# qq456cvb/CPPF2

Hardware: AMD Instinct MI355X
Metric: scenes/sec (1/2/4/8 GPU) at 4096 pts x 20k tuples; 5deg5cm match vs ref (higher is better)
Workload: dtype f32

## Files before the change

### cppf2_amd/_lib.py

```python
from __future__ import annotations

import ctypes as C
import os

_PKG = os.path.dirname(os.path.abspath(__file__))
LIB_PATH = os.path.join(_PKG, "libcppf_hip.so")
if os.environ.get("CPPF_LIB"):
    LIB_PATH = os.path.abspath(os.environ["CPPF_LIB"])

ABI_VERSION = 11


class CppfError(RuntimeError):
    pass


class SceneGrid(C.Structure):
    _fields_ = [("c0", C.c_float * 3), ("g", C.c_int32 * 3), ("ncell", C.c_int32), ("flags", C.c_int32)]


class SceneResult(C.Structure):
    _fields_ = [("argmax", C.c_int64), ("t", C.c_double * 3), ("R", C.c_double * 9), ("scale", C.c_float * 3),
                ("peak", C.c_uint32), ("up_idx", C.c_int32), ("right_idx", C.c_int32), ("kept", C.c_int32),
                ("up_count", C.c_float), ("right_count", C.c_float), ("flags", C.c_int32), ("ncell", C.c_int32), ("pad_", C.c_int32 * 3)]


class ReslayerSplit16Args(C.Structure):
    _fields_ = [("x", C.c_void_p), ("ldx", C.c_int64), ("k_in", C.c_int32),
                ("out", C.c_void_p), ("ldo", C.c_int64), ("n_out", C.c_int32), ("rows", C.c_int64),
                ("wq", C.c_void_p), ("wq_bytes", C.c_int64), ("b1", C.c_void_p), ("b0", C.c_void_p), ("chain", C.c_int32),
                ("weight_scale", C.c_float),
                ("first_out", C.c_void_p), ("ld_first", C.c_int64),
                ("gidx", C.c_void_p), ("slots", C.c_int32), ("table", C.c_void_p), ("fdim", C.c_int32),
                ("logit_prior", C.c_void_p), ("uniforms", C.c_void_p), ("bins", C.c_void_p),
                ("stream", C.c_void_p), ("mode", C.c_int32), ("ld_table", C.c_int64), ("sched", C.c_void_p),
                ("prior_pos", C.c_void_p), ("prior_inv_sigma", C.c_float)]


assert C.sizeof(SceneGrid) == 32
assert C.sizeof(SceneResult) == 160

_p = C.c_void_p
_i = C.c_int
_i32 = C.c_int32
_i64 = C.c_int64
_u64 = C.c_uint64
_f = C.c_float
_d = C.c_double

STABLE = {
    "cppf_version": (_i, []),
    "cppf_last_error_string": (C.c_char_p, []),
# ... 49 lines not shown
}

EXPERIMENTAL = {
    "cppf_shot352_from_normals": (_i, [_i, _p, _p, _i64, _p, _f, _p, _p, _p, _i64, _p]),
    "cppf_cast_f16": (_i, [_p, _p, _i64, _p]),
    "cppf_encode_tuples_shot_f16": (_i, [_i, _p, _p, _p, _i, _p, _i, _p, _p, _i64, _p, _p]),
    "cppf_encode_tuples_dino": (_i, [_i, _p, _i, _i, _p, _p, _p, _p, _i64, _p, _i, _i, _p]),
    "cppf_kept_rows": (_i, [_i, _p, _p, _p, _i, _p, _p]),
    "cppf_reslayer128": (_i, [_p, _i64, _p, _p, _p, _p]),
    "cppf_encode_tuples_shot_heads": (_i, [_i, _p, _p, _p, _i, _p, _p, _i64, _p, _i, _p, _p]),
    "cppf_reslayer_split_gather": (_i, [_p, _i64, _i, _p, _i, _p, _i, _p, _i64, _i, _i64, _p, _i64, _p, _p, _i, _p, _p]),
    "cppf_encode_tuples_coord_heads": (_i, [_i, _p, _p, _i, _p, _p, _i64, _p, _i32, _p, _p]),
    "cppf_reslayer_split_sumgather": (_i, [_p, _i64, _i32, _p, _i32, _p, _i64, _p, _i64, _i32, _i64, _p, _i64, _p, _p, _i32, _p, _p]),
    "cppf_reslayer_split16_stream_bytes": (_i64, [_i32, _i32, _i32, _i32]),
    "cppf_reslayer_split16": (_i, [_p]),
    "cppf_reslayer_split_debug_grid": (_i, [_i32]),
    "cppf_decode_bins_prior": (_i, [_i, _p, _p, _i, _p, _p, _p, _i, _p, _p, _i64, _p, _p, _p, _p, _p, _p, _p]),
    "cppf_reslayer_split_decode_prior": (_i, [_p, _i64, _i, _i64, _p, _i64, _p, _p, _p, _p, C.c_float, _p, _p, _p, _p]),
}

SIGNATURES = dict(STABLE, **EXPERIMENTAL)

CALLED = set()


class _Traced:
    def __init__(self, lib):
        self._lib = lib
        for name in SIGNATURES:
            setattr(self, name, self._wrap(name, getattr(lib, name)))
# ... 42 lines not shown
```

### cppf2_amd/csrc/cppf_mlp_split.hip

```cpp
#include "cppf_common.h"
#include <atomic>
#include <mutex>
#include <type_traits>

typedef float f32x16 __attribute__((ext_vector_type(16)));
typedef float f32x4 __attribute__((ext_vector_type(4)));
typedef __bf16 bf16x8 __attribute__((ext_vector_type(8)));

__host__ __device__ constexpr int rs_waves(int nt) { return nt >= 6 ? 4 : 8; }
#define RS_RESLAYER 0
#define RS_LINEAR 1
#define RS_SUMGATHER 2
#define RS_ENCODE 3
#define RS_SUMENCODE 5
__host__ __device__ constexpr int rs_waves_mode(int nt, int mode) { return mode == RS_LINEAR ? 8 : rs_waves(nt); }
__host__ __device__ constexpr int rs_stage_tiles(int mode) { return 16; }
__host__ __device__ constexpr int rs_wgs_per_cu(int mode) { return 1; }
#define RS_FRAG_BYTES 1024
__host__ __device__ constexpr int rs_stage_bytes(int stg) { return stg * 3 * RS_FRAG_BYTES; }
__host__ __device__ constexpr int rs_tile_bytes(int pc) { return pc * RS_FRAG_BYTES; }

#ifndef RS_DEEP_PREFETCH
#define RS_DEEP_PREFETCH 0
#endif
// ... 73 lines not shown
  acc = rs_mfma<PC>(a.l, b.h, acc);
  acc = rs_mfma<PC>(a.h, b.l, acc);
  if (PC == 3) {
    acc = rs_mfma<PC>(a.m, b.m, acc);
    acc = rs_mfma<PC>(a.m, b.h, acc);
    acc = rs_mfma<PC>(a.h, b.m, acc);
  }
  acc = rs_mfma<PC>(a.h, b.h, acc);
}

__host__ __device__ constexpr int rs_waitcnt(int vm, int lgkm) {
  return (vm & 15) | ((vm >> 4) << 14) | (7 << 4) | ((lgkm & 15) << 8);
}
#define RS_WAIT(vm, lgkm) __builtin_amdgcn_s_waitcnt(rs_waitcnt(vm, lgkm))

template <int NT, int T0, int WAVES, int PC, bool LIN = false, int STG = 16>
struct RsStream {
  static constexpr int STG_ = STG, SPC0 = rs_spc(T0, STG), SPC1 = rs_spc(NT, STG), STAGE_BYTES = rs_stage_bytes(STG);
  static constexpr int P0 = (SPC0 * T0 * PC + WAVES - 1) / WAVES, P1 = (SPC1 * NT * PC + WAVES - 1) / WAVES;
  static constexpr int PMAX = RS_EXACT_PMAX ? (P0 > P1 ? P0 : P1) : 48 / WAVES;
  int nseg;
  int chunks;
  const char* base;
  char* ring;
  int ks1;
  int seg, pos;
  int64_t off;
  int64_t left;
  int stage;
  int wave, lane;
  const char* p_src;
  char* p_dst;
  int p_last;

  __device__ __forceinline__ void shape(int chain) {
    if (LIN) {
      nseg = chain;
      chunks = chain * ((ks1 + SPC0 - 1) / SPC0);
      return;
    }
    nseg = 2 + 2 * chain;
    chunks = (ks1 + SPC0 - 1) / SPC0 + (1 + 2 * chain) * (2 * NT / SPC1);
  }
  __device__ __forceinline__ void plan(int st) {
    p_dst = ring + st * STAGE_BYTES;
    if (left <= 0) {
      p_src = base + lane * 16;
      p_last = 0;
      return;
    }
    const bool first = LIN || seg == 0;
    const int tiles = first ? T0 : NT;
    const int spc = first ? SPC0 : SPC1;
    const int steps = first ? ks1 : 2 * NT;
    const int ns = steps - pos < spc ? steps - pos : spc;
    const int pieces = ns * tiles * PC;
    p_src = base + off + lane * 16;
    p_last = pieces - 1;
    off += (int64_t)pieces * RS_FRAG_BYTES;
    pos += ns;
    if (pos == steps) {
      pos = 0;
      if (++seg == nseg) {
        seg = 0;
        off = 0;
      }
    }
    --left;
  }
// ... 146 lines not shown
      const int step = c * SPC + i, nx = (step + 1 < 2 * NS) ? step + 1 : step;
      RsFrag bn = b;
      rs_step<NTILES, PREFETCH, Stream::PMAX, PC>(dst, w + i * NTILES * PC * 64, b,
                                [&](int p) {
                                  if (step + 1 < 2 * NS) {
                                    const float s0 = src[nx >> 1][8 * (nx & 1) + 2 * p], s1 = src[nx >> 1][8 * (nx & 1) + 2 * p + 1];
                                    rs_split_pair<PC, true>(PC == 2 ? s0 * bs : s0, PC == 2 ? s1 * bs : s1, bn.h[p], bn.m[p], bn.l[p]);
                                  }
                                },
                                [&](int q) { if (i == 0) ws.piece(q); });
      b = bn;
    }
  }
}

__device__ __forceinline__ void rs_load_tile(f32x16& acc, const float* v, int g) {
#pragma unroll
  for (int q = 0; q < 4; ++q) {
    const f32x4 t = *reinterpret_cast<const f32x4*>(v + 8 * q + 4 * g);
    acc[4 * q + 0] = t.x; acc[4 * q + 1] = t.y; acc[4 * q + 2] = t.z; acc[4 * q + 3] = t.w;
  }
}

__device__ __forceinline__ void rs_load_tile_scaled(f32x16& acc, const float* v, int g, float sc) {
#pragma unroll
  for (int q = 0; q < 4; ++q) {
    const f32x4 t = *reinterpret_cast<const f32x4*>(v + 8 * q + 4 * g);
    acc[4 * q + 0] = t.x * sc; acc[4 * q + 1] = t.y * sc; acc[4 * q + 2] = t.z * sc; acc[4 * q + 3] = t.w * sc;
  }
}
// ... 175 lines not shown
#pragma unroll
    for (int c = 0; c < 3; ++c) v[3 * q + c] = p[PI_[q]][c] - p[PJ_[q]][c];
  v[30] = 0.0f; v[31] = 0.0f;
#pragma unroll
  for (int s = 0; s < 2; ++s) {
    f32x4 lo, hi;
    lo.x = g ? v[16 * s + 8] : v[16 * s + 0]; lo.y = g ? v[16 * s + 9] : v[16 * s + 1];
    lo.z = g ? v[16 * s + 10] : v[16 * s + 2]; lo.w = g ? v[16 * s + 11] : v[16 * s + 3];
    hi.x = g ? v[16 * s + 12] : v[16 * s + 4]; hi.y = g ? v[16 * s + 13] : v[16 * s + 5];
    hi.z = g ? v[16 * s + 14] : v[16 * s + 6]; hi.w = g ? v[16 * s + 15] : v[16 * s + 7];
    *reinterpret_cast<f32x4*>(slots + s * 2048 + lane * 16) = lo;
    *reinterpret_cast<f32x4*>(slots + s * 2048 + 1024 + lane * 16) = hi;
  }
}

template <int NT, bool PROJ, bool GATHER, bool DECODE = false, int PC = 3, int MODE = RS_RESLAYER>
__global__ __launch_bounds__(64 * rs_waves_mode(NT, MODE), rs_wgs_per_cu(MODE)) void reslayer_split_kernel(const float* x, int64_t ldx, int k_in, float* out,
                                                                              int64_t ldo, int64_t rows,
                                                                              const char* __restrict__ wq,
                                                                              const float* __restrict__ b1,
                                                                              const float* __restrict__ b0, int chain,
                                                                              RsGather ga, RsDecode dc, RsTap tap, float wscale) {
  const float bs = (PC == 2) ? 1.0f / wscale : 1.0f;
  constexpr int WAVES = rs_waves_mode(NT, MODE), THREADS = 64 * WAVES, BLOCK_ROWS = 32 * WAVES;
  constexpr int T0 = PROJ ? 2 * NT : NT;
  constexpr bool LIN = MODE == RS_LINEAR;
  static_assert(!LIN || (!PROJ && !GATHER && !DECODE), "a plain Linear has one product");
  constexpr bool SUMG = MODE == RS_SUMGATHER || MODE == RS_SUMENCODE;
  constexpr bool LOCAL_IDX = MODE == RS_ENCODE || MODE == RS_SUMENCODE;
  static_assert(!SUMG || (PROJ && !GATHER), "the table sums stand for columns of a projection layer's input");
  static_assert(MODE != RS_ENCODE || (GATHER && !DECODE), "RS_ENCODE is a form of the gathering launch");
  constexpr bool PF = RS_DEEP_PREFETCH && WAVES == 4;
  extern __shared__ __attribute__((aligned(16))) char s_ring[];
  const int lane = threadIdx.x & 63;
  const int wave = __builtin_amdgcn_readfirstlane(threadIdx.x >> 6);
  const int r = lane & 31, g = lane >> 5;
  const int ks1 = (k_in + 15) >> 4;
  const int64_t nblocks = (rows + BLOCK_ROWS - 1) / BLOCK_ROWS;
  int64_t bfirst = blockIdx.x, bstride = gridDim.x, bend = nblocks;
  if (RS_XCD_BLOCKS && (gridDim.x & 7) == 0 && nblocks >= 64) {
    const int64_t xcd = blockIdx.x & 7;
    bfirst = nblocks * xcd / 8 + (blockIdx.x >> 3);
    bend = nblocks * (xcd + 1) / 8;
    bstride = gridDim.x >> 3;
  }
  int* const sched = ga.sched;
  const bool dyn = sched != nullptr && !LIN;
  int* const s_claim = reinterpret_cast<int*>(s_ring + 2 * rs_stage_bytes(rs_stage_tiles(MODE)) + WAVES * 3 * 2048 + (2 + chain) * 32 * NT * 4);
  if (dyn) { bfirst = blockIdx.x; bstride = 0; bend = nblocks; }
  const int64_t mine = dyn ? (bfirst < bend ? 1 : 0) : (bend > bfirst ? (bend - bfirst + bstride - 1) / bstride : 0);
  if (dyn && threadIdx.x == 0) rs_claim_store(&s_claim[0], (int)gridDim.x + atomicAdd(&sched[0], 1));

  constexpr int STG = rs_stage_tiles(MODE), RING_BYTES = 2 * rs_stage_bytes(STG);
  RsStream<NT, T0, WAVES, PC, LIN, STG> ws;
  const int64_t seg_bytes = (int64_t)ks1 * T0 * rs_tile_bytes(PC);
  if (LIN) {
    wq += (int64_t)blockIdx.y * chain * seg_bytes;
    b1 = b1 ? b1 + (int64_t)blockIdx.y * chain * 32 * NT : b1;
    out += (int64_t)blockIdx.y * chain * 32 * NT;
  }
  ws.base = wq;
  ws.ring = s_ring;
  ws.ks1 = ks1;
  ws.seg = 0;
  ws.pos = 0;
  ws.off = 0;
  ws.shape(chain);
  ws.left = mine * ws.chunks;
  ws.stage = 0;
  ws.wave = wave;
  ws.lane = lane;
  ws.prime();
  float* s_b1 = reinterpret_cast<float*>(s_ring + RING_BYTES + WAVES * 3 * 2048);
  float* s_b0 = s_b1 + 32 * NT;
  if (LIN) {
    for (int i = threadIdx.x; i < 32 * NT * chain; i += THREADS) s_b1[i] = b1 ? b1[i] : 0.0f;
  } else {
    for (int i = threadIdx.x; i < 32 * NT; i += THREADS) {
      s_b1[i] = b1[i];
      if (PROJ) s_b0[i] = b0[i];
    }
    for (int i = threadIdx.x; i < 32 * NT * chain; i += THREADS) s_b1[2 * 32 * NT + i] = b1[32 * NT + i];
  }
  __syncthreads();

  RsX<GATHER> xs;
  xs.slots = s_ring + RING_BYTES + wave * (3 * 2048);
  xs.k_in = k_in;
  xs.g = g;
  xs.lane = lane;
  xs.table = ga.table;
  xs.head = ga.head;
  xs.fshift = ga.fshift;
  auto row_of = [&](int64_t blk) {
    const int64_t row = blk * BLOCK_ROWS + wave * 32 + r;
    const int64_t rc = row < rows ? row : rows - 1;
    RsRow rw;
// ... 167 lines not shown
      }
    }
#pragma unroll 1
    for (int l = 0; l < chain; ++l) {
      const float* bl = s_b1 + 32 * NT * (2 + l);
#pragma unroll
      for (int u = 0; u < NT; ++u) rs_load_tile(h[u], bl + 32 * u, g);
      rs_product_h<NT, NT, PF, PC>(h, o, ws, bs);
#pragma unroll
      for (int u = 0; u < NT; ++u) {
#pragma unroll
        for (int e = 0; e < 16; ++e) h[u][e] = (h[u][e] < 0.0f) ? 0.0f : h[u][e];
      }
      rs_product_h<NT, NT, PF, PC>(o, h, ws, bs);
    }
    if (DECODE) {
      if constexpr (NT == 6) rs_decode_epilogue<NT, PC>(o, dc, in ? row : rows - 1, in, g, bs);
    } else if (in && (!(RS_DBG & 32) || o[0][0] == 1.2345e30f)) {
      float* orow = out + row * ldo + 4 * g;
#pragma unroll
      for (int u = 0; u < NT; ++u) {
#pragma unroll
        for (int q = 0; q < 4; ++q) {
          f32x4 v;
          v.x = o[u][4 * q + 0]; v.y = o[u][4 * q + 1]; v.z = o[u][4 * q + 2]; v.w = o[u][4 * q + 3];
          if (PC == 2) v *= bs;
          *reinterpret_cast<f32x4*>(orow + 32 * u + 8 * q) = v;
        }
      }
    }
    blk = nb;
    if (dyn) {
      next_blk = rs_claim_load(&s_claim[par]);
      par ^= 1;
    }
  }
  RS_WAIT(0, 15);
  if (dyn && threadIdx.x == 0) {
    if (atomicAdd(&sched[1], 1) == (int)gridDim.x - 1) {
      __hip_atomic_store(&sched[0], 0, __ATOMIC_RELAXED, __HIP_MEMORY_SCOPE_AGENT);
      __hip_atomic_store(&sched[1], 0, __ATOMIC_RELAXED, __HIP_MEMORY_SCOPE_AGENT);
    }
  }
}

static int64_t rs_stream_bytes(int32_t k_in, int32_t n_out, int32_t proj, int32_t chain, int pc) {
  if (k_in <= 0 || !(n_out == 64 || n_out == 128 || n_out == 192 || n_out == 256) || chain < 0 || chain > 15) return -1;
  const int64_t nt = n_out / 32, ks1 = (k_in + 15) / 16;
  return (ks1 * (proj ? 2 : 1) + (1 + 2 * (int64_t)chain) * 2 * nt) * nt * rs_tile_bytes(pc);
}

extern "C" int64_t cppf_reslayer_split_stream_bytes(int32_t k_in, int32_t n_out, int32_t proj, int32_t chain) {
  return rs_stream_bytes(k_in, n_out, proj, chain, 3);
}

static std::atomic<int> g_rs_debug_cus{0};
extern "C" int cppf_reslayer_split_debug_grid(int32_t workgroups) {
  g_rs_debug_cus.store(workgroups > 0 ? workgroups : 0);
  return CPPF_OK;
}

static std::atomic<int> g_rs_reserved_cus{0};
extern "C" int cppf_mlp_reserve_cus(int32_t cus) {
  CPPF_CHECK_ARG(cus <= 1024);
  return cus < 0 ? g_rs_reserved_cus.load() : g_rs_reserved_cus.exchange(cus);
}

template <int NT, bool PROJ, bool GATHER = false, bool DECODE = false, int PC = 3, int MODE = RS_RESLAYER>
static int rs_launch(const float* x, int64_t ldx, int k_in, float* out, int64_t ldo, int64_t rows, const char* wq,
                     const float* b1, const float* b0, int chain, int cus, hipStream_t stream, RsGather ga = RsGather(),
                     RsDecode dc = RsDecode(), RsTap tap = RsTap(), float wscale = 1.0f) {
  constexpr int WAVES = rs_waves_mode(NT, MODE), THREADS = 64 * WAVES, BLOCK_ROWS = 32 * WAVES;
  const int64_t nblocks = (rows + BLOCK_ROWS - 1) / BLOCK_ROWS;
  const int forced = g_rs_debug_cus.load();
  if (forced > 0) cus = forced;
  else cus = cus - g_rs_reserved_cus.load() > cus / 2 ? cus - g_rs_reserved_cus.load() : (cus + 1) / 2;
  cus *= rs_wgs_per_cu(MODE);
  const unsigned grid = (unsigned)(nblocks < cus ? nblocks : cus);
  unsigned gy = 1;
  if (MODE == RS_LINEAR && (int64_t)grid * 2 <= cus) {
    for (int d = chain; d >= 1; --d)
      if (chain % d == 0 && (int64_t)grid * d <= cus) { gy = (unsigned)d; break; }
    chain /= (int)gy;
  }
  const int lds_bytes = 2 * rs_stage_bytes(rs_stage_tiles(MODE)) + WAVES * 3 * 2048 + (MODE == RS_LINEAR ? chain : 2 + chain) * 32 * NT * 4 + 16;
  if (lds_bytes > 160 * 1024 / rs_wgs_per_cu(MODE)) {
    snprintf(g_cppf_err, sizeof(g_cppf_err), "reslayer_split: %d bytes of LDS for the biases of this launch (too many column groups)", lds_bytes);
    return CPPF_EINVAL;
  }
  {
    static std::mutex mu;
    static bool done[64] = {false};
    int dev = 0;
    CPPF_HIP(hipGetDevice(&dev));
    std::lock_guard<std::mutex> lock(mu);
    if (!done[dev & 63]) {
      CPPF_HIP(hipFuncSetAttribute((const void*)reslayer_split_kernel<NT, PROJ, GATHER, DECODE, PC, MODE>,
                                   hipFuncAttributeMaxDynamicSharedMemorySize, 160 * 1024));
      done[dev & 63] = true;
    }
  }
  hipLaunchKernelGGL((reslayer_split_kernel<NT, PROJ, GATHER, DECODE, PC, MODE>), dim3(grid, gy), dim3(THREADS), lds_bytes, stream, x,
                     ldx, k_in, out, ldo, rows, wq, b1, b0, chain, ga, dc, tap, wscale);
  CPPF_LAUNCH_CHECK();
  return CPPF_OK;
}

static int rs_cus() {
  int dev = 0, n_cu = 0;
  if (hipGetDevice(&dev) != hipSuccess || hipDeviceGetAttribute(&n_cu, hipDeviceAttributeMultiprocessorCount, dev) != hipSuccess) return 256;
  return n_cu > 0 ? n_cu : 256;
}

static int rs_dispatch(const float* x, int64_t ldx, int32_t k_in, float* out, int64_t ldo, int32_t n_out, int64_t rows,
                       const void* wq, int64_t wq_bytes, const float* b1, const float* b0, int32_t chain, RsTap tap,
                       int32_t* sched, void* stream, const char* fn) {
  if (!(x && out && wq && b1 && rows >= 0) || !(k_in > 0 && (k_in & 7) == 0 && ldx >= k_in && (ldx & 3) == 0 && (ldo & 3) == 0 && ldo >= n_out) ||
      !(n_out == 64 || n_out == 128 || n_out == 192 || n_out == 256) || !(b0 != nullptr || k_in == n_out) ||
// ... 209 lines not shown
  if (rows == 0) return CPPF_OK;
  RsGather ga;
  ga.gidx = idx;
  ga.table = tables;
  ga.slots = k;
  ga.tld = ld_tables;
  ga.pts = pts;
  ga.pt_off = pt_off;
  ga.tup_off = tup_off;
  ga.B = B;
  ga.sched = sched;
  return rs_launch<4, true, false, false, 3, RS_SUMENCODE>(nullptr, 0, 32, out, ldo, rows, static_cast<const char*>(wq), b1, b0, chain,
                                                           rs_cus(), (hipStream_t)stream, ga);
}

extern "C" int64_t cppf_reslayer_split16_stream_bytes(int32_t k_in, int32_t n_out, int32_t proj, int32_t chain) {
  return rs_stream_bytes(k_in, n_out, proj, chain, 2);
}

static RsGather rs16_gather(const CppfReslayerSplit16Args& a) {
  RsGather ga;
  ga.sched = a.sched;
  return ga;
}

template <int NT, bool PROJ>
static int rs16_plain(const CppfReslayerSplit16Args& a, int n_cu, RsTap tap) {
  return rs_launch<NT, PROJ, false, false, 2>(a.x, a.ldx, a.k_in, a.out, a.ldo, a.rows, static_cast<const char*>(a.wq), a.b1, a.b0,
                                              a.chain, n_cu, (hipStream_t)a.stream, rs16_gather(a), RsDecode(), tap, a.weight_scale);
}
// ... 88 lines not shown
```

### cppf2_amd/models.py

```python
from __future__ import annotations

import os
from itertools import combinations

import torch
import torch.nn as nn
import torch.nn.functional as F

from . import ops


class ResLayer(nn.Module):

    def __init__(self, dim_in, dim_out):
        super().__init__()
        self.fc1 = nn.Linear(dim_in, dim_out)
        self.fc2 = nn.Linear(dim_out, dim_out)
        self.fc0 = nn.Linear(dim_in, dim_out) if dim_in != dim_out else None

    def forward(self, x):
        skip = x if self.fc0 is None else self.fc0(x)
        return self.fc2(F.relu(self.fc1(x))) + skip


# ... 136 lines not shown
        if MLP_ARITH == "split16":
            sc = f16_scale(w1t, w0t, w2t, *[w for pair in chain for w in pair])
            wq = pack_split(w1t.t(), None if w0t is None else w0t.t(), w2t.t(), k_in, chain=chain, arith="f16x2", scale=sc)
            hit = (stamp, (wq, (biases * sc).contiguous(), None if b0 is None else (b0 * sc).contiguous(), sc))
        else:
            wq = pack_split(w1t.t(), None if w0t is None else w0t.t(), w2t.t(), k_in, chain=chain)
            hit = (stamp, (wq, biases.contiguous(), b0, 1.0))
        cache[key] = hit
    return hit[1]


def _chain_len(cache, key, stamp, compute):
    hit = cache.get(key)
    if hit is None or hit[0] != stamp:
        hit = (stamp, compute())
        cache[key] = hit
    return hit[1]


def fused_stack(seq, x, keep_input=False, gather=None, decode=None, tail=None):
    tap_at, cross = None, None
    if isinstance(seq, (tuple, list)):
        seq_a, seq_b = seq
        plan_a, c_a = _fused_plan(seq_a)
        assert c_a is None, "the first stack must end in a projection layer"
        plan_b, c = _fused_plan(seq_b)
        plan = plan_a + plan_b
        tap_at = len(plan_a) - 1
        cross = seq_b._fused_plan_cache[0]
        seq = seq_b
# ... 23 lines not shown
            assert _kernel_arith() and w0t is not None and w1t.shape[1] == 128 and k_in % 8 == 0, "table-fed first layer: see sum_supported"
            w1t, w0t = fold.w1_heads.t(), fold.w0_heads.t()
        else:
            k_in = heads.shape[1] + (source.k if source is not None else gidx.shape[1]) * table.shape[1]
            assert _kernel_arith() and w0t is not None and w1t.shape == (k_in, 128), "gathered first layer: see gather_supported"
        cache = _entry_cache(entry)

        def gather_chain():
            n = 0
            while (1 + n < len(plan) and plan[1 + n][2] is None and n < 15 and plan[1 + n][0].shape == (128, 128)):
                n += 1
            n = cut(0, n)
            return 0 if tap_at == 0 else n
        chain = _chain_len(cache, ("gather-chain", k_in, tap_at), cross, gather_chain)
        crossing = tap_at is not None and chain > tap_at
        stamp = (cross if crossing else None, None if fold is None else fold.stamp)
        wq, bb1, bb0, sc = _packed(cache, (k_in, chain, crossing, fold is not None), w1t, w0t, w2t, k_in, plan[1:1 + chain], b1, b0,
                                   stamp=stamp, add=None if fold is None else (fold.b1_add, fold.b0_add))
        if fold is not None and source is not None:
            x = ops.reslayer_split_sumencode(source, table, wq, bb1, bb0, 128, chain=chain)
        elif fold is not None:
            x = ops.reslayer_split_sumgather(heads, gidx, table, wq, bb1, bb0, 128, chain=chain,
                                             scale=sc if MLP_ARITH == "split16" else None)
        elif MLP_ARITH == "split16":
            x = ops.reslayer_split16(heads, wq, bb1, bb0, 128, sc, chain=chain, gather=(gidx, table))
        elif source is not None:
            x = ops.reslayer_split_encode(source, table, wq, bb1, bb0, 128, chain=chain)
        else:
            x = ops.reslayer_split_gather(heads, gidx, table, wq, bb1, bb0, 128, chain=chain)
        li = 1 + chain
# ... 15 lines not shown
        if (_kernel_arith() and x.dtype == torch.float32 and x.stride(1) == 1 and x.stride(0) % 4 == 0
                and x.data_ptr() % 16 == 0 and x.shape[1] >= w1t.shape[0]
                and ops.reslayer_split_supported(x.shape[1], n_out, w0t is not None)):
            cache = _entry_cache(entry)
            ahead = tap_at is not None and tap_at >= li

            def plain_chain(li=li, n_out=n_out, w0t=w0t):
                n = 0
                while (li + 1 + n < len(plan) and plan[li + 1 + n][2] is None and n < 15
                       and plan[li + 1 + n][0].shape == (n_out, n_out)
                       and ops.reslayer_split_supported(x.shape[1], n_out, w0t is not None, n + 1)):
                    n += 1
                return cut(li, n)
            chain = _chain_len(cache, ("chain", x.shape[1], tap_at if ahead else None), cross if ahead else None, plain_chain)
            crossing = tap_at is not None and li <= tap_at < li + chain
            wq, bb1, bb0, sc = _packed(cache, (x.shape[1], chain, crossing), w1t, w0t, w2t, x.shape[1],
                                       plan[li + 1:li + 1 + chain], b1, b0, stamp=cross if crossing else None)
            out = None
            if w0t is None and li == 0 and keep_input:
                out = torch.empty_like(x)
            if w0t is None and out is None and tapped is not None and x.data_ptr() == tapped.data_ptr():
                out = torch.empty_like(x)
            tap_buf = None
            if tap_at == li and chain > 0:
                tap_buf = torch.empty((x.shape[0], n_out), dtype=torch.float32, device=x.device)
                if w0t is None and out is None:
                    out = torch.empty_like(x)
            if MLP_ARITH == "split16":
                x = ops.reslayer_split16(x, wq, bb1, bb0, n_out, sc, out=out, chain=chain, tap=tap_buf)
            else:
# ... 318 lines not shown
```

### cppf2_amd/ops.py

```python
from __future__ import annotations

import ctypes as C
import math

import numpy as np
import torch

from . import _lib
from ._lib import CppfError, SceneGrid, SceneResult

_L = _lib.load()

BMM_SIZE = 100000


def _dev():
    if not torch.cuda.is_available():
        raise CppfError("cppf2_amd needs a HIP device (torch.cuda.is_available() is False); there is no CPU fallback")
    return torch.device("cuda", torch.cuda.current_device())


def _stream():
    return C.c_void_p(torch.cuda.current_stream().cuda_stream)

# ... 391 lines not shown
    assert heads.is_cuda and heads.dtype == torch.float32 and heads.dim() == 2
    assert gidx.dtype == torch.int32 and gidx.is_contiguous() and table.dtype == torch.float32 and table.is_contiguous()
    rows = gidx.shape[0]
    out = torch.empty((rows, n_out), dtype=torch.float32, device=heads.device)
    b1 = b1.contiguous()
    b0 = b0.contiguous()
    assert b1.numel() == (1 + chain) * n_out
    ld_heads = heads.stride(0) if heads.shape[1] else 0
    _lib.check(_L.cppf_reslayer_split_gather(_p(heads if heads.shape[1] else table), ld_heads, heads.shape[1], _p(gidx), gidx.shape[1], _p(table),
                                             table.shape[1], _p(out), out.stride(0), n_out, rows, _p(wq),
                                             wq.numel() * wq.element_size(), _p(b1), _p(b0), int(chain), _sched(), _stream()),
               "cppf_reslayer_split_gather")
    return out


class TupleSource:

    def __init__(self, points, point_idxs_all, normal=None, pt_off=None, tup_off=None):
        dev = _dev()
        self.pts = _t(points, torch.float32, dev)
        self.nrm = None if normal is None else _t(normal, torch.float32, dev)
        self.idx = _t(point_idxs_all, torch.int32, dev)
        T, self.k = self.idx.shape
        if pt_off is None:
            pt_off, tup_off = _offsets([self.pts.shape[0]], dev), _offsets([T], dev)
        self.pt_off, self.tup_off = pt_off, tup_off
        self.B = pt_off.numel() - 1
        npair = self.k * (self.k - 1) // 2
        self.shape = (T, npair * 4 if normal is not None else (npair * 3 + 7) // 8 * 8)

# ... 375 lines not shown
```

### include/cppf_hip_experimental.h

```cpp
#ifndef CPPF_HIP_EXPERIMENTAL_H_
#define CPPF_HIP_EXPERIMENTAL_H_

#include "cppf_hip.h"

#ifdef __cplusplus
extern "C" {
#endif

int cppf_decode_bins_prior(int B, const float* logits, const float* logit_prior, int nb, const float* uniforms,
                           const float* pts, const int32_t* idx, int k, const int32_t* pt_off, const int32_t* tup_off,
                           int64_t total_tuples, const double* h_axes, int32_t* bins, float* scaled, float* scale,
                           float* tr, float* rot, void* stream);
int cppf_reslayer_split_decode_prior(const float* x, int64_t ldx, int32_t k_in, int64_t rows, const void* wq, int64_t wq_bytes,
                                     const float* b1, const float* b0, const float* logit_prior, const float* prior_pos,
                                     float prior_inv_sigma, const float* uniforms, int32_t* bins, int32_t* sched, void* stream);

int cppf_shot352_from_normals(int B, const float* pts, const int32_t* pt_off, int64_t total_points,
                              const float* normals, float shot_r, float* out_shot, float* out_rf,
                              void* workspace, int64_t workspace_bytes, void* stream);

int cppf_cast_f16(const float* x, void* out_half, int64_t n, void* stream);

int cppf_encode_tuples_shot_f16(int B, const float* pts, const float* normals, const void* feat_half, int feat_dim,
                                const int32_t* idx, int k, const int32_t* pt_off, const int32_t* tup_off,
// ... 30 lines not shown
  const void* wq; int64_t wq_bytes; const float* b1; const float* b0; int32_t chain;
  float weight_scale;
  float* first_out; int64_t ld_first;
  const int32_t* gidx; int32_t slots; const float* table; int32_t fdim;
  const float* logit_prior; const float* uniforms; int32_t* bins;
  void* stream;
  int32_t mode;
  int64_t ld_table;
  int32_t* sched;
  const float* prior_pos;
  float prior_inv_sigma;
} CppfReslayerSplit16Args;
int64_t cppf_reslayer_split16_stream_bytes(int32_t k_in, int32_t n_out, int32_t proj, int32_t chain);
int cppf_reslayer_split16(const CppfReslayerSplit16Args* args);

int cppf_reslayer_split_debug_grid(int32_t workgroups);

#ifdef __cplusplus
}
#endif
#endif
```

Baseline: 5279.

## Fuse 128->64 tail residual layer and narrow output head into the reslayer chain kernel

Extends the split-precision residual MLP kernel so that, after its chain of 128-wide residual blocks, it also runs a following 128->64 projection residual layer in the same launch. On gathered rows it can further apply the final 64->3 narrow layer in a scalar FMA epilogue and scatter the results. The goal is to remove separate kernel launches and the global-memory round trips for the intermediate activations. In exchange it adds more weight-stream segments, extra LDS for tail biases, and register pressure from the larger fused body. It is enabled by default through CHAIN_TAILS when the layer shapes match.

```diff
diff --git a/cppf2_amd/_lib.py b/cppf2_amd/_lib.py
--- a/cppf2_amd/_lib.py
+++ b/cppf2_amd/_lib.py
@@ -36,6 +36,17 @@
                 ("stream", C.c_void_p), ("mode", C.c_int32), ("ld_table", C.c_int64), ("sched", C.c_void_p),
                 ("prior_pos", C.c_void_p), ("prior_inv_sigma", C.c_float)]
 
+
+
+class ReslayerSplitChainArgs(C.Structure):
+    _fields_ = [("x", C.c_void_p), ("ldx", C.c_int64), ("k_in", C.c_int32),
+                ("gidx", C.c_void_p), ("slots", C.c_int32), ("table", C.c_void_p), ("fdim", C.c_int32),
+                ("n_out", C.c_int32), ("n_tail", C.c_int32), ("rows", C.c_int64),
+                ("wq", C.c_void_p), ("wq_bytes", C.c_int64), ("b1", C.c_void_p), ("b0", C.c_void_p), ("chain", C.c_int32),
+                ("out", C.c_void_p), ("ldo", C.c_int64),
+                ("n_narrow", C.c_int32), ("narrow_w", C.c_void_p),
+                ("scatter_rows", C.c_void_p), ("valid_count", C.c_void_p), ("per_group", C.c_int32),
+                ("sched", C.c_void_p), ("stream", C.c_void_p)]
 
 assert C.sizeof(SceneGrid) == 32
 assert C.sizeof(SceneResult) == 160
@@ -115,6 +126,7 @@
     "cppf_reslayer_split_sumgather": (_i, [_p, _i64, _i32, _p, _i32, _p, _i64, _p, _i64, _i32, _i64, _p, _i64, _p, _p, _i32, _p, _p]),
     "cppf_reslayer_split16_stream_bytes": (_i64, [_i32, _i32, _i32, _i32]),
     "cppf_reslayer_split16": (_i, [_p]),
+    "cppf_reslayer_split_chain": (_i, [_p]),
     "cppf_reslayer_split_debug_grid": (_i, [_i32]),
     "cppf_decode_bins_prior": (_i, [_i, _p, _p, _i, _p, _p, _p, _i, _p, _p, _i64, _p, _p, _p, _p, _p, _p, _p]),
     "cppf_reslayer_split_decode_prior": (_i, [_p, _i64, _i, _i64, _p, _i64, _p, _p, _p, _p, C.c_float, _p, _p, _p, _p]),
diff --git a/cppf2_amd/csrc/cppf_mlp_split.hip b/cppf2_amd/csrc/cppf_mlp_split.hip
--- a/cppf2_amd/csrc/cppf_mlp_split.hip
+++ b/cppf2_amd/csrc/cppf_mlp_split.hip
@@ -111,11 +111,17 @@
 }
 #define RS_WAIT(vm, lgkm) __builtin_amdgcn_s_waitcnt(rs_waitcnt(vm, lgkm))
 
-template <int NT, int T0, int WAVES, int PC, bool LIN = false, int STG = 16>
+__host__ __device__ constexpr int rs_pieces(int tiles, int waves, int pc, int stg) {
+  return tiles > 0 ? (rs_spc(tiles, stg) * tiles * pc + waves - 1) / waves : 0;
+}
+__host__ __device__ constexpr int rs_max(int a, int b) { return a > b ? a : b; }
+template <int NT, int T0, int WAVES, int PC, bool LIN = false, int STG = 16, int NT2 = 0>
 struct RsStream {
   static constexpr int STG_ = STG, SPC0 = rs_spc(T0, STG), SPC1 = rs_spc(NT, STG), STAGE_BYTES = rs_stage_bytes(STG);
+  static constexpr int SPC2 = rs_spc(NT2 > 0 ? 2 * NT2 : 1, STG), SPC3 = rs_spc(NT2 > 0 ? NT2 : 1, STG);
   static constexpr int P0 = (SPC0 * T0 * PC + WAVES - 1) / WAVES, P1 = (SPC1 * NT * PC + WAVES - 1) / WAVES;
-  static constexpr int PMAX = RS_EXACT_PMAX ? (P0 > P1 ? P0 : P1) : 48 / WAVES;
+  static constexpr int P23 = rs_max(rs_pieces(2 * NT2, WAVES, PC, STG), rs_pieces(NT2, WAVES, PC, STG));
+  static constexpr int PMAX = RS_EXACT_PMAX ? rs_max(P0 > P1 ? P0 : P1, P23) : 48 / WAVES;
   int nseg;
   int chunks;
   const char* base;
@@ -136,8 +142,9 @@
       chunks = chain * ((ks1 + SPC0 - 1) / SPC0);
       return;
     }
-    nseg = 2 + 2 * chain;
+    nseg = 2 + 2 * chain + (NT2 > 0 ? 2 : 0);
     chunks = (ks1 + SPC0 - 1) / SPC0 + (1 + 2 * chain) * (2 * NT / SPC1);
+    if (NT2 > 0) chunks += 2 * NT / SPC2 + 2 * NT2 / SPC3;
   }
   __device__ __forceinline__ void plan(int st) {
     p_dst = ring + st * STAGE_BYTES;
@@ -147,9 +154,15 @@
       return;
     }
     const bool first = LIN || seg == 0;
-    const int tiles = first ? T0 : NT;
-    const int spc = first ? SPC0 : SPC1;
-    const int steps = first ? ks1 : 2 * NT;
+    int tiles = first ? T0 : NT;
+    int spc = first ? SPC0 : SPC1;
+    int steps = first ? ks1 : 2 * NT;
+    if (NT2 > 0 && seg >= nseg - 2) {
+      const bool w2 = seg == nseg - 1;
+      tiles = w2 ? NT2 : 2 * NT2;
+      spc = w2 ? SPC3 : SPC2;
+      steps = w2 ? 2 * NT2 : 2 * NT;
+    }
     const int ns = steps - pos < spc ? steps - pos : spc;
     const int pieces = ns * tiles * PC;
     p_src = base + off + lane * 16;
@@ -326,6 +339,109 @@
   }
 }
 
+__device__ __forceinline__ void rs_x_order(float (&v)[8], const f32x16& t, int q, int g) {
+#pragma unroll
+  for (int c = 0; c < 4; ++c) {
+    const float a = t[4 * q + c], b = t[4 * q + 4 + c];
+    const float pa = __shfl_xor(a, 32), pb = __shfl_xor(b, 32);
+    v[c] = g ? pb : a;
+    v[4 + c] = g ? b : pa;
+  }
+}
+
+template <int NS, int NTILES, bool PREFETCH, int PC, class Stream>
+__device__ __forceinline__ void rs_product_hx(f32x16 (&dst)[NTILES], const f32x16 (&src)[NS], Stream& ws, int g) {
+  static_assert(PC == 3, "bf16 triples only");
+  constexpr int SPC = rs_spc(NTILES, Stream::STG_);
+  static_assert((2 * NS) % SPC == 0, "whole chunks");
+  float xv[8];
+  rs_x_order(xv, src[0], 0, g);
+  RsFrag b = rs_split<PC>(xv);
+#pragma unroll
+  for (int c = 0; c < 2 * NS / SPC; ++c) {
+    const u32x4* w = ws.template acquire<0>();
+#pragma unroll
+    for (int i = 0; i < SPC; ++i) {
+      const int step = c * SPC + i, nx = (step + 1 < 2 * NS) ? step + 1 : step;
+      float nv[8];
+      rs_x_order(nv, src[nx >> 1], 2 * (nx & 1), g);
+      RsFrag bn = b;
+      rs_step<NTILES, PREFETCH, Stream::PMAX, PC>(dst, w + i * NTILES * PC * 64, b,
+                                [&](int p) {
+                                  if (step + 1 < 2 * NS) rs_split_pair<PC, true>(nv[2 * p], nv[2 * p + 1], bn.h[p], bn.m[p], bn.l[p]);
+                                },
+                                [&](int q) { if (i == 0) ws.piece(q); });
+      b = bn;
+    }
+  }
+}
+
+struct RsNarrow {
+  const float* w = nullptr;
+  const int32_t* scatter_rows = nullptr;
+  const int32_t* valid_count = nullptr;
+  int per_group = 0;
+  float* out = nullptr;
+  int64_t ldo = 0;
+};
+
+template <int NS, int N>
+__device__ __forceinline__ void rs_narrow_epilogue(const f32x16 (&y)[NS], const RsNarrow& nw, const float* __restrict__ w, int row, bool in, int g) {
+  constexpr int K = 32 * NS;
+  int opaque = 0;
+  asm volatile("" : "+s"(opaque));
+  const float* w1 = w + opaque;
+  const float* w0 = w1 + N * K;
+  const float* b1 = w0 + N * K;
+  const float* b0 = b1 + N;
+  const float* w2 = b0 + N;
+  float h[N], s[N];
+#pragma unroll
+  for (int n = 0; n < N; ++n) {
+    h[n] = b1[n];
+    s[n] = b0[n];
+  }
+#pragma unroll
+  for (int t = 0; t < NS; ++t) {
+#pragma unroll
+    for (int q = 0; q < 4; ++q) {
+      float x[8];
+#pragma unroll
+      for (int c = 0; c < 4; ++c) {
+        const float v = y[t][4 * q + c], p = __shfl_xor(v, 32);
+        x[c] = g ? p : v;
+        x[4 + c] = g ? v : p;
+      }
+      const int k0 = 32 * t + 8 * q;
+#pragma unroll
+      for (int j = 0; j < 8; ++j) {
+#pragma unroll
+        for (int n = 0; n < N; ++n) {
+          h[n] = fmaf(x[j], w1[n * K + k0 + j], h[n]);
+          s[n] = fmaf(x[j], w0[n * K + k0 + j], s[n]);
+        }
+      }
+      __builtin_amdgcn_sched_barrier(0);
+    }
+  }
+#pragma unroll
+  for (int n = 0; n < N; ++n) h[n] = (h[n] < 0.0f) ? 0.0f : h[n];
+  int64_t dst = row;
+  if (nw.scatter_rows) {
+    if (nw.valid_count && row % nw.per_group >= nw.valid_count[row / nw.per_group]) in = false;
+    dst = in ? (int64_t)nw.scatter_rows[row] : 0;
+  }
+  if (in && g == 0) {
+#pragma unroll
+    for (int n = 0; n < N; ++n) {
+      float o = s[n];
+#pragma unroll
+      for (int m = 0; m < N; ++m) o = fmaf(h[m], w2[n * N + m], o);
+      nw.out[dst * nw.ldo + n] = o;
+    }
+  }
+}
+
 __device__ __forceinline__ void rs_load_tile(f32x16& acc, const float* v, int g) {
 #pragma unroll
   for (int q = 0; q < 4; ++q) {
@@ -531,13 +647,11 @@
   }
 }
 
-template <int NT, bool PROJ, bool GATHER, bool DECODE = false, int PC = 3, int MODE = RS_RESLAYER>
-__global__ __launch_bounds__(64 * rs_waves_mode(NT, MODE), rs_wgs_per_cu(MODE)) void reslayer_split_kernel(const float* x, int64_t ldx, int k_in, float* out,
-                                                                              int64_t ldo, int64_t rows,
-                                                                              const char* __restrict__ wq,
-                                                                              const float* __restrict__ b1,
-                                                                              const float* __restrict__ b0, int chain,
-                                                                              RsGather ga, RsDecode dc, RsTap tap, float wscale) {
+template <int NT, bool PROJ, bool GATHER, bool DECODE, int PC, int MODE, int NT2, int NARROW>
+__device__ __forceinline__ void reslayer_split_body(const float* x, int64_t ldx, int k_in, float* out, int64_t ldo, int64_t rows,
+                                                    const char* __restrict__ wq, const float* __restrict__ b1,
+                                                    const float* __restrict__ b0, int chain, RsGather ga, RsDecode dc, RsTap tap,
+                                                    float wscale, RsNarrow nw, const float* __restrict__ nw_w) {
   const float bs = (PC == 2) ? 1.0f / wscale : 1.0f;
   constexpr int WAVES = rs_waves_mode(NT, MODE), THREADS = 64 * WAVES, BLOCK_ROWS = 32 * WAVES;
   constexpr int T0 = PROJ ? 2 * NT : NT;
@@ -547,6 +661,8 @@
   constexpr bool LOCAL_IDX = MODE == RS_ENCODE || MODE == RS_SUMENCODE;
   static_assert(!SUMG || (PROJ && !GATHER), "the table sums stand for columns of a projection layer's input");
   static_assert(MODE != RS_ENCODE || (GATHER && !DECODE), "RS_ENCODE is a form of the gathering launch");
+  static_assert(NT2 == 0 || (PC == 3 && MODE == RS_RESLAYER && !DECODE && 2 * NT2 <= NT), "a tail layer at most as wide as the launch");
+  static_assert(NARROW == 0 || NT2 > 0, "the narrow epilogue follows a tail layer");
   constexpr bool PF = RS_DEEP_PREFETCH && WAVES == 4;
   extern __shared__ __attribute__((aligned(16))) char s_ring[];
   const int lane = threadIdx.x & 63;
@@ -563,13 +679,14 @@
   }
   int* const sched = ga.sched;
   const bool dyn = sched != nullptr && !LIN;
-  int* const s_claim = reinterpret_cast<int*>(s_ring + 2 * rs_stage_bytes(rs_stage_tiles(MODE)) + WAVES * 3 * 2048 + (2 + chain) * 32 * NT * 4);
+  int* const s_claim = reinterpret_cast<int*>(s_ring + 2 * rs_stage_bytes(rs_stage_tiles(MODE)) + WAVES * 3 * 2048 + (2 + chain) * 32 * NT * 4 +
+                                              2 * 32 * NT2 * 4);
   if (dyn) { bfirst = blockIdx.x; bstride = 0; bend = nblocks; }
   const int64_t mine = dyn ? (bfirst < bend ? 1 : 0) : (bend > bfirst ? (bend - bfirst + bstride - 1) / bstride : 0);
   if (dyn && threadIdx.x == 0) rs_claim_store(&s_claim[0], (int)gridDim.x + atomicAdd(&sched[0], 1));
 
   constexpr int STG = rs_stage_tiles(MODE), RING_BYTES = 2 * rs_stage_bytes(STG);
-  RsStream<NT, T0, WAVES, PC, LIN, STG> ws;
+  RsStream<NT, T0, WAVES, PC, LIN, STG, NT2> ws;
   const int64_t seg_bytes = (int64_t)ks1 * T0 * rs_tile_bytes(PC);
   if (LIN) {
     wq += (int64_t)blockIdx.y * chain * seg_bytes;
@@ -598,6 +715,8 @@
       if (PROJ) s_b0[i] = b0[i];
     }
     for (int i = threadIdx.x; i < 32 * NT * chain; i += THREADS) s_b1[2 * 32 * NT + i] = b1[32 * NT + i];
+    for (int i = threadIdx.x; i < 2 * 32 * NT2; i += THREADS)
+      s_b1[(2 + chain) * 32 * NT + i] = b1[(1 + chain) * 32 * NT + i];
   }
   __syncthreads();
 
@@ -795,7 +914,35 @@
       }
       rs_product_h<NT, NT, PF, PC>(o, h, ws, bs);
     }
-    if (DECODE) {
+    if constexpr (NT2 > 0) {
+      f32x16 (&t1)[2 * NT2] = *reinterpret_cast<f32x16 (*)[2 * NT2]>(&acc[0]);
+      f32x16 (&h2)[NT2] = *reinterpret_cast<f32x16 (*)[NT2]>(&acc[0]);
+      f32x16 (&o2)[NT2] = *reinterpret_cast<f32x16 (*)[NT2]>(&acc[NT2]);
+      const float* bt = s_b1 + 32 * NT * (2 + chain);
+#pragma unroll
+      for (int u = 0; u < 2 * NT2; ++u) rs_load_tile(t1[u], bt + 32 * u, g);
+      rs_product_hx<NT, 2 * NT2, PF, PC>(t1, o, ws, g);
+#pragma unroll
+      for (int u = 0; u < NT2; ++u) {
+#pragma unroll
+        for (int e = 0; e < 16; ++e) h2[u][e] = (h2[u][e] < 0.0f) ? 0.0f : h2[u][e];
+      }
+      rs_product_h<NT2, NT2, PF, PC>(o2, h2, ws, bs);
+      if constexpr (NARROW > 0) {
+        rs_narrow_epilogue<NT2, NARROW>(o2, nw, nw_w, (int)(in ? row : rows - 1), in, g);
+      } else if (in) {
+        float* orow = out + row * ldo + 4 * g;
+#pragma unroll
+        for (int u = 0; u < NT2; ++u) {
+#pragma unroll
+          for (int q = 0; q < 4; ++q) {
+            f32x4 v;
+            v.x = o2[u][4 * q + 0]; v.y = o2[u][4 * q + 1]; v.z = o2[u][4 * q + 2]; v.w = o2[u][4 * q + 3];
+            *reinterpret_cast<f32x4*>(orow + 32 * u + 8 * q) = v;
+          }
+        }
+      }
+    } else if (DECODE) {
       if constexpr (NT == 6) rs_decode_epilogue<NT, PC>(o, dc, in ? row : rows - 1, in, g, bs);
     } else if (in && (!(RS_DBG & 32) || o[0][0] == 1.2345e30f)) {
       float* orow = out + row * ldo + 4 * g;
@@ -825,6 +972,27 @@
   }
 }
 
+template <int NT, bool PROJ, bool GATHER, bool DECODE = false, int PC = 3, int MODE = RS_RESLAYER>
+__global__ __launch_bounds__(64 * rs_waves_mode(NT, MODE), rs_wgs_per_cu(MODE)) void reslayer_split_kernel(const float* x, int64_t ldx, int k_in, float* out,
+                                                                              int64_t ldo, int64_t rows,
+                                                                              const char* __restrict__ wq,
+                                                                              const float* __restrict__ b1,
+                                                                              const float* __restrict__ b0, int chain,
+                                                                              RsGather ga, RsDecode dc, RsTap tap, float wscale) {
+  reslayer_split_body<NT, PROJ, GATHER, DECODE, PC, MODE, 0, 0>(x, ldx, k_in, out, ldo, rows, wq, b1, b0, chain, ga, dc, tap, wscale,
+                                                               RsNarrow(), nullptr);
+}
+
+template <int NT, bool PROJ, bool GATHER, int NT2, int NARROW>
+__global__ __launch_bounds__(64 * rs_waves(NT), 1) void reslayer_split_chain_kernel(const float* x, int64_t ldx, int k_in, float* out, int64_t ldo,
+                                                                                 int64_t rows, const char* __restrict__ wq,
+                                                                                 const float* __restrict__ b1, const float* __restrict__ b0,
+                                                                                 int chain, RsGather ga, RsNarrow nw,
+                                                                                 const float* __restrict__ nw_w) {
+  reslayer_split_body<NT, PROJ, GATHER, false, 3, RS_RESLAYER, NT2, NARROW>(x, ldx, k_in, out, ldo, rows, wq, b1, b0, chain, ga, RsDecode(),
+                                                                           RsTap(), 1.0f, nw, nw_w);
+}
+
 static int64_t rs_stream_bytes(int32_t k_in, int32_t n_out, int32_t proj, int32_t chain, int pc) {
   if (k_in <= 0 || !(n_out == 64 || n_out == 128 || n_out == 192 || n_out == 256) || chain < 0 || chain > 15) return -1;
   const int64_t nt = n_out / 32, ks1 = (k_in + 15) / 16;
@@ -847,10 +1015,10 @@
   return cus < 0 ? g_rs_reserved_cus.load() : g_rs_reserved_cus.exchange(cus);
 }
 
-template <int NT, bool PROJ, bool GATHER = false, bool DECODE = false, int PC = 3, int MODE = RS_RESLAYER>
+template <int NT, bool PROJ, bool GATHER = false, bool DECODE = false, int PC = 3, int MODE = RS_RESLAYER, int NT2 = 0, int NARROW = 0>
 static int rs_launch(const float* x, int64_t ldx, int k_in, float* out, int64_t ldo, int64_t rows, const char* wq,
                      const float* b1, const float* b0, int chain, int cus, hipStream_t stream, RsGather ga = RsGather(),
-                     RsDecode dc = RsDecode(), RsTap tap = RsTap(), float wscale = 1.0f) {
+                     RsDecode dc = RsDecode(), RsTap tap = RsTap(), float wscale = 1.0f, RsNarrow nw = RsNarrow()) {
   constexpr int WAVES = rs_waves_mode(NT, MODE), THREADS = 64 * WAVES, BLOCK_ROWS = 32 * WAVES;
   const int64_t nblocks = (rows + BLOCK_ROWS - 1) / BLOCK_ROWS;
   const int forced = g_rs_debug_cus.load();
@@ -864,7 +1032,8 @@
       if (chain % d == 0 && (int64_t)grid * d <= cus) { gy = (unsigned)d; break; }
     chain /= (int)gy;
   }
-  const int lds_bytes = 2 * rs_stage_bytes(rs_stage_tiles(MODE)) + WAVES * 3 * 2048 + (MODE == RS_LINEAR ? chain : 2 + chain) * 32 * NT * 4 + 16;
+  const int lds_bytes = 2 * rs_stage_bytes(rs_stage_tiles(MODE)) + WAVES * 3 * 2048 + (MODE == RS_LINEAR ? chain : 2 + chain) * 32 * NT * 4 +
+                        2 * 32 * NT2 * 4 + 16;
   if (lds_bytes > 160 * 1024 / rs_wgs_per_cu(MODE)) {
     snprintf(g_cppf_err, sizeof(g_cppf_err), "reslayer_split: %d bytes of LDS for the biases of this launch (too many column groups)", lds_bytes);
     return CPPF_EINVAL;
@@ -876,13 +1045,21 @@
     CPPF_HIP(hipGetDevice(&dev));
     std::lock_guard<std::mutex> lock(mu);
     if (!done[dev & 63]) {
-      CPPF_HIP(hipFuncSetAttribute((const void*)reslayer_split_kernel<NT, PROJ, GATHER, DECODE, PC, MODE>,
-                                   hipFuncAttributeMaxDynamicSharedMemorySize, 160 * 1024));
+      if constexpr (NT2 > 0)
+        CPPF_HIP(hipFuncSetAttribute((const void*)reslayer_split_chain_kernel<NT, PROJ, GATHER, NT2, NARROW>,
+                                     hipFuncAttributeMaxDynamicSharedMemorySize, 160 * 1024));
+      else
+        CPPF_HIP(hipFuncSetAttribute((const void*)reslayer_split_kernel<NT, PROJ, GATHER, DECODE, PC, MODE>,
+                                     hipFuncAttributeMaxDynamicSharedMemorySize, 160 * 1024));
       done[dev & 63] = true;
     }
   }
-  hipLaunchKernelGGL((reslayer_split_kernel<NT, PROJ, GATHER, DECODE, PC, MODE>), dim3(grid, gy), dim3(THREADS), lds_bytes, stream, x,
-                     ldx, k_in, out, ldo, rows, wq, b1, b0, chain, ga, dc, tap, wscale);
+  if constexpr (NT2 > 0)
+    hipLaunchKernelGGL((reslayer_split_chain_kernel<NT, PROJ, GATHER, NT2, NARROW>), dim3(grid, gy), dim3(THREADS), lds_bytes, stream, x, ldx,
+                       k_in, out, ldo, rows, wq, b1, b0, chain, ga, nw, nw.w);
+  else
+    hipLaunchKernelGGL((reslayer_split_kernel<NT, PROJ, GATHER, DECODE, PC, MODE>), dim3(grid, gy), dim3(THREADS), lds_bytes, stream, x,
+                       ldx, k_in, out, ldo, rows, wq, b1, b0, chain, ga, dc, tap, wscale);
   CPPF_LAUNCH_CHECK();
   return CPPF_OK;
 }
@@ -1122,6 +1299,57 @@
                                                            rs_cus(), (hipStream_t)stream, ga);
 }
 
+extern "C" int cppf_reslayer_split_chain(const CppfReslayerSplitChainArgs* args) {
+  CPPF_CHECK_ARG(args != nullptr);
+  const CppfReslayerSplitChainArgs& a = *args;
+  const bool gather = a.gidx != nullptr;
+  CPPF_CHECK_ARG(a.wq && a.b1 && a.b0 && a.rows >= 0 && a.chain >= 0 && a.chain <= 15);
+  CPPF_CHECK_ARG(a.n_out == 128 && a.n_tail == 64 && a.n_narrow >= 0 && a.n_narrow <= 8);
+  CPPF_CHECK_ARG((((uintptr_t)a.x | (uintptr_t)a.out | (uintptr_t)a.wq | (uintptr_t)a.table) & 15) == 0 && (a.ldx & 3) == 0);
+  int k_in = a.k_in;
+  RsGather ga;
+  ga.sched = a.sched;
+  if (gather) {
+    CPPF_CHECK_ARG(a.table && a.k_in >= 0 && (a.k_in & 7) == 0 && (a.k_in == 0 || (a.x && a.ldx >= a.k_in)));
+    CPPF_CHECK_ARG(a.slots >= 1 && a.slots <= 8 && a.fdim >= 8 && (a.fdim & (a.fdim - 1)) == 0);
+    ga.gidx = a.gidx;
+    ga.table = a.table;
+    ga.slots = a.slots;
+    ga.head = a.k_in;
+    ga.fshift = __builtin_ctz((unsigned)a.fdim);
+    k_in = a.k_in + a.slots * a.fdim;
+  } else {
+    CPPF_CHECK_ARG(a.x && a.k_in > 0 && (a.k_in & 7) == 0 && a.ldx >= a.k_in);
+  }
+  CPPF_CHECK_ARG(a.wq_bytes == cppf_reslayer_split_stream_bytes(k_in, a.n_out, 1, a.chain) +
+                                   cppf_reslayer_split_stream_bytes(a.n_out, a.n_tail, 1, 0));
+  RsNarrow nw;
+  if (a.n_narrow > 0) {
+    CPPF_CHECK_ARG(a.narrow_w && a.out && a.ldo >= a.n_narrow);
+    CPPF_CHECK_ARG(a.valid_count == nullptr || (a.scatter_rows != nullptr && a.per_group > 0 && a.rows % a.per_group == 0));
+    nw.w = a.narrow_w;
+    nw.scatter_rows = a.scatter_rows;
+    nw.valid_count = a.valid_count;
+    nw.per_group = a.per_group;
+    nw.out = a.out;
+    nw.ldo = a.ldo;
+  } else {
+    CPPF_CHECK_ARG(a.out && (a.ldo & 3) == 0 && a.ldo >= a.n_tail && !a.scatter_rows && !a.valid_count);
+  }
+  if (a.rows == 0) return CPPF_OK;
+  const char* w = static_cast<const char*>(a.wq);
+  hipStream_t st = (hipStream_t)a.stream;
+  const int n_cu = rs_cus();
+  if (a.n_narrow == 3 && gather)
+    return rs_launch<4, true, true, false, 3, RS_RESLAYER, 2, 3>(a.x, a.ldx, k_in, nullptr, 0, a.rows, w, a.b1, a.b0, a.chain, n_cu, st, ga,
+                                                                 RsDecode(), RsTap(), 1.0f, nw);
+  if (a.n_narrow == 0 && !gather)
+    return rs_launch<4, true, false, false, 3, RS_RESLAYER, 2>(a.x, a.ldx, k_in, a.out, a.ldo, a.rows, w, a.b1, a.b0, a.chain, n_cu, st, ga);
+  snprintf(g_cppf_err, sizeof(g_cppf_err), "cppf_reslayer_split_chain: n_narrow = %d with%s gather (kernels: 128 -> 64 on x; 128 -> 64 -> 3 "
+           "on gathered rows)", a.n_narrow, gather ? "" : "out");
+  return CPPF_EUNSUPPORTED;
+}
+
 extern "C" int64_t cppf_reslayer_split16_stream_bytes(int32_t k_in, int32_t n_out, int32_t proj, int32_t chain) {
   return rs_stream_bytes(k_in, n_out, proj, chain, 2);
 }
diff --git a/cppf2_amd/models.py b/cppf2_amd/models.py
--- a/cppf2_amd/models.py
+++ b/cppf2_amd/models.py
@@ -174,6 +174,35 @@
     hit = cache.get(key)
     if hit is None or hit[0] != stamp:
         hit = (stamp, compute())
+        cache[key] = hit
+    return hit[1]
+
+
+CHAIN_TAILS = True
+
+
+def _tail_layer(plan, i):
+    return i < len(plan) and plan[i][2] is not None and tuple(plan[i][0].shape) == (128, 64)
+
+
+def _narrow_layer(plan, i):
+    return (i == len(plan) - 1 and plan[i][2] is not None and plan[i][0].shape[0] == 64 and plan[i][0].shape[1] <= 8)
+
+
+def _chain_packed(plan, li, chain, first, narrow):
+    cache = _entry_cache(plan[li])
+    wq0, bb1, bb0, _ = _packed(cache, *first)
+    t = plan[li + 1 + chain]
+    wq1, tb1, tb0, _ = _packed(_entry_cache(t), (128, 0, False), t[0], t[2], t[4], 128, [], t[1], t[3])
+    key = ("chain-tail", chain, narrow, MLP_ARITH)
+    stamp = (wq0.data_ptr(), bb1.data_ptr(), wq1.data_ptr(), tb1.data_ptr(), tb0.data_ptr())
+    hit = cache.get(key)
+    if hit is None or hit[0] != stamp:
+        nw = None
+        if narrow:
+            e = plan[li + 2 + chain]
+            nw = torch.cat([e[0].t().reshape(-1), e[2].t().reshape(-1), e[1], e[3], e[4].t().reshape(-1)]).float().contiguous()
+        hit = (stamp, (torch.cat([wq0, wq1]).contiguous(), torch.cat([bb1, tb1, tb0]).contiguous(), bb0, nw))
         cache[key] = hit
     return hit[1]
 
@@ -227,6 +256,16 @@
             return 0 if tap_at == 0 else n
         chain = _chain_len(cache, ("gather-chain", k_in, tap_at), cross, gather_chain)
         crossing = tap_at is not None and chain > tap_at
+        if (CHAIN_TAILS and MLP_ARITH == "split" and fold is None and source is None and tap_at is None and decode is None
+                and _tail_layer(plan, 1 + chain) and _narrow_layer(plan, 2 + chain) and gidx.shape[0] < 2 ** 31):
+            wq, bb1, bb0, nw = _chain_packed(plan, 0, chain, ((k_in, chain, False, False), w1t, w0t, w2t, k_in, plan[1:1 + chain], b1, b0, (None, None)),
+                                             True)
+            n = plan[-1][0].shape[1]
+            if tail is not None:
+                narrow = (nw, tail[0], tail[1], tail[2], tail[3])
+            else:
+                narrow = (nw, None, None, 0, torch.empty((gidx.shape[0], n), dtype=torch.float32, device=table.device))
+            return ops.reslayer_split_chain(heads, wq, bb1, bb0, chain, gather=(gidx, table), narrow=narrow)
         stamp = (cross if crossing else None, None if fold is None else fold.stamp)
         wq, bb1, bb0, sc = _packed(cache, (k_in, chain, crossing, fold is not None), w1t, w0t, w2t, k_in, plan[1:1 + chain], b1, b0,
                                    stamp=stamp, add=None if fold is None else (fold.b1_add, fold.b0_add))
@@ -272,6 +311,13 @@
                 return cut(li, n)
             chain = _chain_len(cache, ("chain", x.shape[1], tap_at if ahead else None), cross if ahead else None, plain_chain)
             crossing = tap_at is not None and li <= tap_at < li + chain
+            if (CHAIN_TAILS and MLP_ARITH == "split" and tap_at is None and decode is None and w0t is not None and n_out == 128
+                    and _tail_layer(plan, li + 1 + chain)):
+                wq, bb1, bb0, _ = _chain_packed(plan, li, chain, ((x.shape[1], chain, False), w1t, w0t, w2t, x.shape[1],
+                                                                  plan[li + 1:li + 1 + chain], b1, b0), False)
+                x = ops.reslayer_split_chain(x, wq, bb1, bb0, chain)
+                li += 2 + chain
+                continue
             wq, bb1, bb0, sc = _packed(cache, (x.shape[1], chain, crossing), w1t, w0t, w2t, x.shape[1],
                                        plan[li + 1:li + 1 + chain], b1, b0, stamp=cross if crossing else None)
             out = None
diff --git a/cppf2_amd/ops.py b/cppf2_amd/ops.py
--- a/cppf2_amd/ops.py
+++ b/cppf2_amd/ops.py
@@ -429,6 +429,50 @@
     return out
 
 
+def reslayer_split_chain(x, wq, b1, b0, chain, gather=None, out=None, narrow=None):
+    assert x.is_cuda and x.dtype == torch.float32 and x.dim() == 2 and x.stride(1) == 1
+    b1, b0 = b1.contiguous(), b0.contiguous()
+    assert b1.numel() == (1 + chain) * 128 + 128
+    a = _lib.ReslayerSplitChainArgs()
+    a.k_in = x.shape[1]
+    if gather is not None:
+        gidx, table = gather
+        assert gidx.dtype == torch.int32 and gidx.is_contiguous() and table.dtype == torch.float32 and table.is_contiguous()
+        rows = gidx.shape[0]
+        a.x = (x if x.shape[1] else table).data_ptr()
+        a.ldx = x.stride(0) if x.shape[1] else 0
+        a.gidx, a.slots, a.table, a.fdim = gidx.data_ptr(), gidx.shape[1], table.data_ptr(), table.shape[1]
+    else:
+        rows = x.shape[0]
+        a.x, a.ldx = x.data_ptr(), x.stride(0)
+    if rows == 0:
+        return narrow[4] if narrow is not None else (out if out is not None else torch.empty((0, 64), dtype=torch.float32, device=x.device))
+    a.n_out, a.n_tail, a.rows = 128, 64, rows
+    a.wq, a.wq_bytes = wq.data_ptr(), wq.numel() * wq.element_size()
+    a.b1, a.b0, a.chain = b1.data_ptr(), b0.data_ptr(), int(chain)
+    if narrow is not None:
+        w, scatter_rows, valid_count, per_group, out = narrow
+        n = out.shape[1]
+        assert w.dtype == torch.float32 and w.is_contiguous() and w.numel() == n * (64 + 64 + 2 + n)
+        assert out.dtype == torch.float32 and out.stride(1) == 1
+        if scatter_rows is not None:
+            assert scatter_rows.dtype == torch.int32 and scatter_rows.is_contiguous() and scatter_rows.numel() == rows
+        if valid_count is not None:
+            assert valid_count.dtype == torch.int32 and valid_count.is_contiguous() and valid_count.numel() * per_group == rows
+        a.n_narrow, a.narrow_w = n, w.data_ptr()
+        a.scatter_rows = 0 if scatter_rows is None else scatter_rows.data_ptr()
+        a.valid_count = 0 if valid_count is None else valid_count.data_ptr()
+        a.per_group = int(per_group)
+    elif out is None:
+        out = torch.empty((rows, 64), dtype=torch.float32, device=x.device)
+    assert out.dtype == torch.float32 and out.stride(1) == 1
+    a.out, a.ldo = out.data_ptr(), out.stride(0)
+    a.sched = _sched().value or 0
+    a.stream = _stream().value or 0
+    _lib.check(_L.cppf_reslayer_split_chain(C.byref(a)), "cppf_reslayer_split_chain")
+    return out
+
+
 class TupleSource:
 
     def __init__(self, points, point_idxs_all, normal=None, pt_off=None, tup_off=None):
diff --git a/include/cppf_hip_experimental.h b/include/cppf_hip_experimental.h
--- a/include/cppf_hip_experimental.h
+++ b/include/cppf_hip_experimental.h
@@ -68,6 +68,18 @@
 int64_t cppf_reslayer_split16_stream_bytes(int32_t k_in, int32_t n_out, int32_t proj, int32_t chain);
 int cppf_reslayer_split16(const CppfReslayerSplit16Args* args);
 
+typedef struct CppfReslayerSplitChainArgs {
+  const float* x; int64_t ldx; int32_t k_in;
+  const int32_t* gidx; int32_t slots; const float* table; int32_t fdim;
+  int32_t n_out; int32_t n_tail; int64_t rows;
+  const void* wq; int64_t wq_bytes; const float* b1; const float* b0; int32_t chain;
+  float* out; int64_t ldo;
+  int32_t n_narrow; const float* narrow_w;
+  const int32_t* scatter_rows; const int32_t* valid_count; int32_t per_group;
+  int32_t* sched; void* stream;
+} CppfReslayerSplitChainArgs;
+int cppf_reslayer_split_chain(const CppfReslayerSplitChainArgs* args);
+
 int cppf_reslayer_split_debug_grid(int32_t workgroups);
 
 #ifdef __cplusplus
```

After: 5309 (median of 6 runs). No clear change (+0.6%).
